# ultralytics/yolov5

Hardware: NVIDIA H100
Metric: images/sec @640 (forward + NMS) (higher is better)
Workload: dtype bf16

## Files before the change

### yolov5_b200/csrc/common.cuh

```cuda
#pragma once
#include <cuda.h>
#include <cuda_bf16.h>
#include <cuda_fp16.h>
#include <cuda_runtime.h>
#include <stdint.h>
#include <stdio.h>

namespace y5 {

__device__ __forceinline__ uint32_t smem_u32(const void* p) { return static_cast<uint32_t>(__cvta_generic_to_shared(p)); }

__device__ __forceinline__ bool elect_one() {
    uint32_t pred = 0;
    asm volatile(
        "{\n\t.reg .pred P;\n\t"
        "elect.sync _|P, 0xffffffff;\n\t"
        "selp.b32 %0, 1, 0, P;\n\t}"
        : "=r"(pred));
    return pred != 0;
}

__device__ __forceinline__ void mbar_init(uint64_t* bar, uint32_t count) {
    asm volatile("mbarrier.init.shared::cta.b64 [%0], %1;" ::"r"(smem_u32(bar)), "r"(count) : "memory");
}
__device__ __forceinline__ void fence_barrier_init() { asm volatile("fence.mbarrier_init.release.cluster;" ::: "memory"); }
__device__ __forceinline__ void fence_proxy_async_smem() { asm volatile("fence.proxy.async.shared::cta;" ::: "memory"); }

__device__ __forceinline__ void mbar_arrive(uint64_t* bar) {
    asm volatile("{\n\t.reg .b64 st;\n\tmbarrier.arrive.shared::cta.b64 st, [%0];\n\t}" ::"r"(smem_u32(bar)) : "memory");
}
__device__ __forceinline__ void mbar_arrive_expect_tx(uint64_t* bar, uint32_t bytes) {
    asm volatile("{\n\t.reg .b64 st;\n\tmbarrier.arrive.expect_tx.shared::cta.b64 st, [%0], %1;\n\t}" ::"r"(smem_u32(bar)),
                 "r"(bytes)
                 : "memory");
}
__device__ __forceinline__ bool mbar_try_wait(uint64_t* bar, uint32_t parity) {
    uint32_t ok;
    asm volatile(
        "{\n\t.reg .pred P;\n\t"
        "mbarrier.try_wait.parity.shared::cta.b64 P, [%1], %2;\n\t"
        "selp.b32 %0, 1, 0, P;\n\t}"
        : "=r"(ok)
        : "r"(smem_u32(bar)), "r"(parity)
        : "memory");
    return ok != 0;
}
__device__ __forceinline__ bool mbar_try_wait_hint(uint64_t* bar, uint32_t parity, uint32_t ns) {
    uint32_t ok;
    asm volatile(
        "{\n\t.reg .pred P;\n\t"
        "mbarrier.try_wait.parity.shared::cta.b64 P, [%1], %2, %3;\n\t"
        "selp.b32 %0, 1, 0, P;\n\t}"
        : "=r"(ok)
        : "r"(smem_u32(bar)), "r"(parity), "r"(ns)
        : "memory");
    return ok != 0;
}
__device__ __forceinline__ void mbar_wait(uint64_t* bar, uint32_t parity) {
    if (mbar_try_wait(bar, parity)) return;
    uint32_t spins = 0;
    while (!mbar_try_wait_hint(bar, parity, 20000u)) {
        if (++spins > 200000u) __trap();
    }
}

__device__ __forceinline__ void tma_prefetch_desc(const CUtensorMap* m) {
    asm volatile("prefetch.tensormap [%0];" ::"l"(reinterpret_cast<uint64_t>(m)) : "memory");
}
__device__ __forceinline__ void tma_load_2d(const CUtensorMap* m, uint64_t* bar, void* dst, int c0, int c1) {
    asm volatile(
        "cp.async.bulk.tensor.2d.shared::cluster.global.mbarrier::complete_tx::bytes [%0], [%1, {%3, %4}], [%2];" ::"r"(
            smem_u32(dst)),
        "l"(reinterpret_cast<uint64_t>(m)), "r"(smem_u32(bar)), "r"(c0), "r"(c1)
        : "memory");
}
__device__ __forceinline__ void tma_load_4d(const CUtensorMap* m, uint64_t* bar, void* dst, int c0, int c1, int c2, int c3) {
    asm volatile(
        "cp.async.bulk.tensor.4d.shared::cluster.global.mbarrier::complete_tx::bytes [%0], [%1, {%3, %4, %5, %6}], [%2];" ::"r"(
            smem_u32(dst)),
        "l"(reinterpret_cast<uint64_t>(m)), "r"(smem_u32(bar)), "r"(c0), "r"(c1), "r"(c2), "r"(c3)
        : "memory");
}
__device__ __forceinline__ void tma_load_2d_mcast(const CUtensorMap* m, uint64_t* bar, void* dst, int c0, int c1, uint16_t mask) {
    asm volatile(
        "cp.async.bulk.tensor.2d.shared::cluster.global.mbarrier::complete_tx::bytes.multicast::cluster"
        " [%0], [%1, {%3, %4}], [%2], %5;" ::"r"(smem_u32(dst)),
        "l"(reinterpret_cast<uint64_t>(m)), "r"(smem_u32(bar)), "r"(c0), "r"(c1), "h"(mask)
        : "memory");
}
__device__ __forceinline__ uint32_t mapa_u32(const void* p, uint32_t rank) {
    uint32_t r;
    asm volatile("mapa.shared::cluster.u32 %0, %1, %2;" : "=r"(r) : "r"(smem_u32(p)), "r"(rank));
    return r;
}
__device__ __forceinline__ void mbar_arrive_cluster(uint32_t bar_addr) {
    asm volatile("mbarrier.arrive.release.cluster.shared::cluster.b64 _, [%0];" ::"r"(bar_addr) : "memory");
}
__device__ __forceinline__ uint32_t cluster_ctarank() { uint32_t r; asm volatile("mov.u32 %0, %%cluster_ctarank;" : "=r"(r)); return r; }
__device__ __forceinline__ uint32_t cluster_nctarank() { uint32_t r; asm volatile("mov.u32 %0, %%cluster_nctarank;" : "=r"(r)); return r; }
__device__ __forceinline__ void cluster_sync_all() {
    asm volatile("barrier.cluster.arrive.release.aligned;" ::: "memory");
    asm volatile("barrier.cluster.wait.acquire.aligned;" ::: "memory");
}
__device__ __forceinline__ void tma_load_im2col_4d(const CUtensorMap* m, uint64_t* bar, void* dst, int c, int w, int h,
                                                   int n, uint16_t off_w, uint16_t off_h) {
    asm volatile(
        "cp.async.bulk.tensor.4d.shared::cluster.global.im2col.mbarrier::complete_tx::bytes"
        " [%0], [%1, {%3, %4, %5, %6}], [%2], {%7, %8};" ::"r"(smem_u32(dst)),
        "l"(reinterpret_cast<uint64_t>(m)), "r"(smem_u32(bar)), "r"(c), "r"(w), "r"(h), "r"(n), "h"(off_w), "h"(off_h)
        : "memory");
}
__device__ __forceinline__ void tma_store_2d(const CUtensorMap* m, const void* src, int c0, int c1) {
    asm volatile("cp.async.bulk.tensor.2d.global.shared::cta.bulk_group [%0, {%2, %3}], [%1];" ::"l"(
                     reinterpret_cast<uint64_t>(m)),
                 "r"(smem_u32(src)), "r"(c0), "r"(c1)
                 : "memory");
}
__device__ __forceinline__ void tma_store_4d(const CUtensorMap* m, const void* src, int c0, int c1, int c2, int c3) {
    asm volatile("cp.async.bulk.tensor.4d.global.shared::cta.bulk_group [%0, {%2, %3, %4, %5}], [%1];" ::"l"(
                     reinterpret_cast<uint64_t>(m)),
                 "r"(smem_u32(src)), "r"(c0), "r"(c1), "r"(c2), "r"(c3)
                 : "memory");
}
__device__ __forceinline__ void tma_store_commit() { asm volatile("cp.async.bulk.commit_group;" ::: "memory"); }
__device__ __forceinline__ void tma_store_wait_read0() { asm volatile("cp.async.bulk.wait_group.read 0;" ::: "memory"); }
__device__ __forceinline__ void tma_store_wait_all() { asm volatile("cp.async.bulk.wait_group 0;" ::: "memory"); }

__device__ __forceinline__ uint32_t gmma_desc_hi(uint32_t row_bytes) {
    const uint32_t layout = row_bytes == 128 ? 1u : (row_bytes == 64 ? 2u : 3u);
    return (((8u * row_bytes) >> 4) & 0x3FFFu) | (layout << 30);
}
__device__ __forceinline__ uint32_t gmma_desc_lo(uint32_t saddr) { return ((saddr >> 4) & 0x3FFFu) | (1u << 16); }
__device__ __forceinline__ uint64_t gmma_desc(uint32_t lo, uint32_t hi) { return (static_cast<uint64_t>(hi) << 32) | lo; }

__device__ __forceinline__ void wgmma_fence() { asm volatile("wgmma.fence.sync.aligned;" ::: "memory"); }
__device__ __forceinline__ void wgmma_commit() { asm volatile("wgmma.commit_group.sync.aligned;" ::: "memory"); }
template <int N>
__device__ __forceinline__ void wgmma_wait() { asm volatile("wgmma.wait_group.sync.aligned %0;" ::"n"(N) : "memory"); }
template <int N>
__device__ __forceinline__ void fence_regs(float (&d)[N]) {
#pragma unroll
    for (int i = 0; i < N; ++i) asm volatile("" : "+f"(d[i])::"memory");
}

template <uint32_t R>
__device__ __forceinline__ void setmaxnreg_dec() { asm volatile("setmaxnreg.dec.sync.aligned.u32 %0;" ::"n"(R)); }
template <uint32_t R>
__device__ __forceinline__ void setmaxnreg_inc() { asm volatile("setmaxnreg.inc.sync.aligned.u32 %0;" ::"n"(R)); }

__device__ __forceinline__ void griddep_wait() { asm volatile("griddepcontrol.wait;" ::: "memory"); }
__device__ __forceinline__ void griddep_launch_dependents() { asm volatile("griddepcontrol.launch_dependents;" ::: "memory"); }

__device__ __forceinline__ uint32_t ld_shared_u32(uint32_t addr) {
    uint32_t v;
    asm volatile("ld.shared.b32 %0, [%1];" : "=r"(v) : "r"(addr) : "memory");
    return v;
}
__device__ __forceinline__ void st_shared_u32(uint32_t addr, uint32_t v) {
    asm volatile("st.shared.b32 [%0], %1;" ::"r"(addr), "r"(v) : "memory");
}

__device__ __forceinline__ void named_bar_sync(uint32_t id, uint32_t nthreads) {
    asm volatile("bar.sync %0, %1;" ::"r"(id), "r"(nthreads) : "memory");
}

#ifndef Y5_SILU_EXACT
__device__ __forceinline__ float silu_f(float x) {
    const float h = 0.5f * x;
    float t;
    asm("tanh.approx.f32 %0, %1;" : "=f"(t) : "f"(h));
    return fmaf(h, t, h);
}
__device__ __forceinline__ float silu_from_half(float h) {
    float t;
    asm("tanh.approx.f32 %0, %1;" : "=f"(t) : "f"(h));
    return fmaf(h, t, h);
}
#else
__device__ __forceinline__ float silu_f(float x) { return __fdividef(x, 1.0f + __expf(-x)); }
// ... 36 lines not shown
```

### yolov5_b200/csrc/conv_gemm.cu

```cuda
#include <cmath>
#include <cstdio>
#include <cstdlib>
#include <cstring>
#include <mutex>
#include <type_traits>

#include "../../include/y5b200.h"
#include "common.cuh"
#include "host_util.h"
#include "wgmma.cuh"

namespace y5 {

constexpr int kBlockM = 128;
constexpr int kConsumers = 2;
constexpr int kConsumerThreads = 128 * kConsumers;
constexpr int kThreads = 128 + kConsumerThreads;
constexpr int kMaxStages = 8;
constexpr int kHeadN = 128;
constexpr int kHeadMaxNo = 8192;
constexpr int kHeadMaxNc = 4096;

__host__ __device__ inline int head_stage_cols(int no) { return no < kHeadN ? no : kHeadN; }

enum AMode { A_LINEAR = 0, A_IM2COL = 1, A_PATCH = 2 };

struct ConvParams {
    int M, N;
    int num_m_tiles;
    int num_m_super, num_n_tiles;
    int kh, kw, c_chunks;
    int block_k;
    int a_mode;
    int Ho, Wo, HoWo, stride, pad_h, pad_w;
    int tw, th, tiles_x, tiles_y;
    int b_grouped;
    int patch_pw;
    int cluster_n;
    uint32_t stg_bytes;
    int tma_epi;
    uint32_t b_sub_bytes;
    float rcp_per_img, rcp_tiles_x, rcp_HoWo, rcp_Wo;
    int a_stages, b_stages;
    uint32_t a_sub_bytes, a_stage_bytes, b_stage_bytes;
    int is_bf16, act;
    const float* bias;
    int bias_n;
    void* out;
    int out_pitch;
    const void* res;
    int res_pitch;
    void* raw;
    void* z;
    int na, no, nc, nx, z_rows, z_row0;
    float det_stride;
    float anchor_wh[8];
    float slope;
};

struct SmemLayout {
    uint32_t off_a, off_b, off_out, off_bias, off_bars, total;
};

__host__ __device__ inline SmemLayout smem_layout(int epi, int no, int bias_n, int a_stages, int b_stages, uint32_t a_bytes,
                                                   uint32_t b_bytes, uint32_t stg_bytes) {
    SmemLayout L;
    uint32_t o = 0;
    L.off_a = o;
    o += a_stages * a_bytes;
    L.off_b = o;
    o += b_stages * b_bytes;
    o = (o + 1023) & ~1023u;
    L.off_out = o;
    if (epi == 1) o += 4 * ((kBlockM * head_stage_cols(no) * 2 + 1023) & ~1023u);
    else o += stg_bytes;
    L.off_bias = o;
    o += ((bias_n + 3) & ~3) * 4;
    o = (o + 7) & ~7u;
    L.off_bars = o;
    o += (4 * kMaxStages + 2) * 8;
    L.total = o;
    return L;
}

__device__ __forceinline__ int fdiv(int n, int d, float rd) {
    if (n >= (1 << 23)) return n / d;
    int q = __float2int_rz(__int2float_rz(n) * rd);
    const int r = n - q * d;
    if (r >= d) ++q;
    else if (r < 0) --q;
    return q;
}

template <int BLOCK_N>
struct EpiBox {
    static constexpr int kRB = BLOCK_N * 2 < 128 ? BLOCK_N * 2 : 128;
    static constexpr int kCols = kRB / 2;
    static constexpr int kNB = BLOCK_N / kCols;
    static constexpr uint32_t kBytes = 64u * kRB;
};
struct EpiOrigin {
    int x, y, img;
};
__device__ __forceinline__ EpiOrigin epi_origin(const ConvParams& p, int mt, int wg) {
    if (p.a_mode != A_PATCH) return {0, mt * kBlockM + 64 * wg, 0};
    const int per_img = p.tiles_x * p.tiles_y;
    const int img = fdiv(mt, per_img, p.rcp_per_img);
    const int rem = mt - img * per_img;
    const int ty = fdiv(rem, p.tiles_x, p.rcp_tiles_x);
    const int x = (rem - ty * p.tiles_x) * p.tw, y = ty * p.th;
    return p.tw > 64 ? EpiOrigin{x + 64 * wg, y, img} : EpiOrigin{x, y + wg * (64 / p.tw), img};
}

template <int BLOCK_N, int MT, int KS, bool BF16>
__device__ __forceinline__ void mma_batch(float (&acc)[MT][BLOCK_N / 2], uint32_t a_lo, uint32_t a_sub16, uint32_t a_hi, uint32_t b_lo,
                                          uint32_t b_hi, uint32_t scale_first) {
    wgmma_fence();
#pragma unroll
    for (int k = 0; k < KS; ++k)
#pragma unroll
        for (int mi = 0; mi < MT; ++mi)
            Wgmma<BLOCK_N>::template run<BF16, 0, 0>(acc[mi], gmma_desc(a_lo + mi * a_sub16 + 2 * k, a_hi), gmma_desc(b_lo + 2 * k, b_hi),
                                                     k == 0 ? scale_first : 1u);
    wgmma_commit();
}

template <int BLOCK_N, int EPI, int MT, bool OPT, bool BF16>
__global__ void __launch_bounds__(kThreads, 1)
conv_gemm_kernel(const __grid_constant__ CUtensorMap tmA, const __grid_constant__ CUtensorMap tmB, const __grid_constant__ CUtensorMap tmO,
                 const __grid_constant__ CUtensorMap tmR, const ConvParams p) {
    static_assert(MT * BLOCK_N <= 256, "accumulators: at most 128 fp32 registers per consumer thread");
    constexpr bool kConv = EPI != 1;
    constexpr bool kLeaky = EPI == 2;
    constexpr int kAcc = BLOCK_N / 2;
    using Box = EpiBox<BLOCK_N>;
    const bool tma_epi = kConv && !OPT && p.tma_epi;

    extern __shared__ __align__(1024) uint8_t smem_raw[];
    uint8_t* smem = reinterpret_cast<uint8_t*>((reinterpret_cast<uintptr_t>(smem_raw) + 1023) & ~uintptr_t(1023));
    const SmemLayout L = smem_layout(EPI, p.no, p.bias_n, p.a_stages, p.b_stages, p.a_stage_bytes, p.b_stage_bytes, p.stg_bytes);
// ... 41 lines not shown
    griddep_launch_dependents();

    const int nn = p.num_n_tiles;
    const int num_tiles = ((p.num_m_super + csize - 1) / csize) * nn;
    const int tile0 = blockIdx.x / csize, tile_step = gridDim.x / csize;
    const uint32_t row_bytes = p.block_k * 2;
    const bool patch = p.a_mode == A_PATCH;
    const bool wide = OPT && p.patch_pw > 0;
    const int grp = wide ? p.kh * p.kw : (patch ? p.kh : 1);
    const int num_groups = wide ? p.c_chunks : (patch ? p.c_chunks * p.kw : p.kh * p.kw * p.c_chunks);

    if (warp < 4) {
        setmaxnreg_dec<56>();
    }
    if (warp == 0) {
        int as = 0, bs = 0;
        uint32_t aph = 0, bph = 0, sph = 0;
        for (int tile = tile0; tile < num_tiles; tile += tile_step) {
            const int ms = (tile / nn) * csize + static_cast<int>(crank);
            const int n0 = (tile - (tile / nn) * nn) * BLOCK_N;
            int img[MT], y0[MT], x0[MT];
#pragma unroll
            for (int mi = 0; mi < MT; ++mi) {
                const int mt = ms * MT + mi;
                img[mi] = y0[mi] = x0[mi] = 0;
                if (p.a_mode == A_IM2COL) {
                    const int m0 = mt * kBlockM;
                    img[mi] = fdiv(m0, p.HoWo, p.rcp_HoWo);
                    const int rem = m0 - img[mi] * p.HoWo;
                    const int oy = fdiv(rem, p.Wo, p.rcp_Wo);
                    y0[mi] = oy * p.stride - p.pad_h;
                    x0[mi] = (rem - oy * p.Wo) * p.stride - p.pad_w;
                } else if (patch) {
                    const int per_img = p.tiles_x * p.tiles_y;
                    img[mi] = fdiv(mt, per_img, p.rcp_per_img);
                    const int rem = mt - img[mi] * per_img;
                    const int ty = fdiv(rem, p.tiles_x, p.rcp_tiles_x);
                    y0[mi] = ty * p.th - p.pad_h;
                    x0[mi] = (rem - ty * p.tiles_x) * p.tw - p.pad_w;
                }
            }
            auto issue_group = [&](int cc, int s, int r0) {
                mbar_wait(&a_empty[as], aph ^ 1);
                if (elect_one()) {
                    mbar_arrive_expect_tx(&a_full[as], p.a_stage_bytes);
#pragma unroll
                    for (int mi = 0; mi < MT; ++mi) {
                        uint8_t* a_dst = sA + as * p.a_stage_bytes + mi * p.a_sub_bytes;
                        if (wide) {
                            if (mi == 0) tma_load_4d(&tmA, &a_full[as], a_dst, cc * p.block_k, x0[0], y0[0], img[0]);
                        } else if (p.a_mode == A_LINEAR) tma_load_2d(&tmA, &a_full[as], a_dst, cc * p.block_k, (ms * MT + mi) * kBlockM);
                        else if (p.a_mode == A_IM2COL)
                            tma_load_im2col_4d(&tmA, &a_full[as], a_dst, cc * p.block_k, x0[mi], y0[mi], img[mi], static_cast<uint16_t>(s),
                                               static_cast<uint16_t>(r0));
                        else tma_load_4d(&tmA, &a_full[as], a_dst, cc * p.block_k, x0[mi] + s, y0[mi], img[mi]);
                    }
                }
                __syncwarp();
                if (++as == p.a_stages) { as = 0; aph ^= 1; }
                for (int j = 0; j < grp; ++j) {
                    const int r = patch ? j : r0;
                    const int kb = wide ? j * p.c_chunks + cc : (r * p.kw + s) * p.c_chunks + cc;
                    const bool stage_first = !p.b_grouped || j == 0, stage_last = !p.b_grouped || j == grp - 1;
                    if (stage_first) mbar_wait(&b_empty[bs], bph ^ 1);
                    if (elect_one()) {
                        if (stage_first) mbar_arrive_expect_tx(&b_full[bs], p.b_stage_bytes);
                        uint8_t* b_dst = sB + bs * p.b_stage_bytes + (p.b_grouped ? j * p.b_sub_bytes : 0u);
                        if (csize == 1) tma_load_2d(&tmB, &b_full[bs], b_dst, kb * p.block_k, n0);
                        else {
                            const int slice_rows = BLOCK_N / csize;
                            tma_load_2d_mcast(&tmB, &b_full[bs], b_dst + crank * slice_rows * row_bytes, kb * p.block_k,
                                              n0 + static_cast<int>(crank) * slice_rows, static_cast<uint16_t>((1u << csize) - 1u));
                        }
                    }
                    __syncwarp();
                    if (stage_last && ++bs == p.b_stages) { bs = 0; bph ^= 1; }
                }
            };
            if (wide) {
                for (int cc = 0; cc < p.c_chunks; ++cc) issue_group(cc, 0, 0);
            } else if (patch) {
                for (int cc = 0; cc < p.c_chunks; ++cc)
                    for (int s = 0; s < p.kw; ++s) issue_group(cc, s, 0);
            } else {
                for (int r = 0; r < p.kh; ++r)
                    for (int s = 0; s < p.kw; ++s)
                        for (int cc = 0; cc < p.c_chunks; ++cc) issue_group(cc, s, r);
            }
            if (tma_epi) {
                mbar_wait(stg_free, sph ^ 1);
                if (elect_one()) {
                    if (p.res) {
                        mbar_arrive_expect_tx(res_full, p.stg_bytes);
#pragma unroll 1
                        for (int i = 0; i < kConsumers * MT; ++i) {
                            const EpiOrigin o = epi_origin(p, ms * MT + i % MT, i / MT);
#pragma unroll
                            for (int b = 0; b < Box::kNB; ++b) {
                                uint8_t* dst = stg + (i * Box::kNB + b) * Box::kBytes;
                                if (patch) tma_load_4d(&tmR, res_full, dst, n0 + b * Box::kCols, o.x, o.y, o.img);
                                else tma_load_2d(&tmR, res_full, dst, n0 + b * Box::kCols, o.y);
                            }
                        }
                    } else {
                        mbar_arrive(res_full);
                    }
                }
                __syncwarp();
                sph ^= 1;
            }
        }
    } else if (warp >= 4) {
    setmaxnreg_inc<224>();
    const int wg = (warp >> 2) - 1;
    const int ct = threadIdx.x - 128;
    const int wrow = wg * 64 + (warp & 3) * 16 + (lane >> 2);
    const int ccol = 2 * (lane & 3);
    const bool signal = (threadIdx.x & 127) == 0;
    constexpr bool bf16 = BF16;
    const uint32_t dhi = gmma_desc_hi(row_bytes);
    const uint32_t a_hi = wide ? (dhi & ~0x3FFFu) | (((static_cast<uint32_t>(p.patch_pw) * row_bytes) >> 4) & 0x3FFFu) : dhi;
    const uint32_t a_base = gmma_desc_lo(smem_u32(sA) + (wide ? wg * 8 * p.patch_pw : wg * 64) * row_bytes), b_base = gmma_desc_lo(smem_u32(sB));
    const uint32_t row16 = row_bytes >> 4;
    const uint32_t a_stage16 = p.a_stage_bytes >> 4, b_stage16 = p.b_stage_bytes >> 4, a_sub16 = p.a_sub_bytes >> 4;
    const uint32_t b_sub16 = p.b_sub_bytes >> 4;
    const uint32_t a_shift16 = patch ? (p.tw * row_bytes) >> 4 : 0;
    const int k_steps = p.block_k / 16;
    const int per_img = p.tiles_x * p.tiles_y;
    const int tw_shift = patch ? __ffs(p.tw) - 1 : 0;
    int as = 0, bs = 0, head_set = 0;
    uint32_t aph = 0, bph = 0, rph = 0;
    float acc[MT][kAcc];
#pragma unroll
    for (int mi = 0; mi < MT; ++mi)
#pragma unroll
        for (int i = 0; i < kAcc; ++i) acc[mi][i] = 0.0f;

    int pend_as = 0, pend_bs = 0;
    bool pend_a_last = false, pend_b_last = false;
    auto release_pending = [&]() {
        if (!signal) return;
        if (pend_b_last) {
            if (csize == 1) mbar_arrive(&b_empty[pend_bs]);
            else
                for (int r = 0; r < csize; ++r) mbar_arrive_cluster(mapa_u32(&b_empty[pend_bs], static_cast<uint32_t>(r)));
        }
        if (pend_a_last) mbar_arrive(&a_empty[pend_as]);
    };

    for (int tile = tile0; tile < num_tiles; tile += tile_step) {
        const int ms = (tile / nn) * csize + static_cast<int>(crank);
        const int nt = tile - (tile / nn) * nn;
        const int n0 = nt * BLOCK_N;
        for (int g = 0; g < num_groups; ++g) {
            mbar_wait(&a_full[as], aph);
            const uint32_t a_stage_lo = a_base + as * a_stage16;
            uint32_t a_lo = a_stage_lo;
            for (int j = 0; j < grp; ++j) {
                if (wide) {
                    const int tr = j / p.kw, ts = j - tr * p.kw;
                    a_lo = a_stage_lo + (tr * p.patch_pw + ts) * row16;
                }
                const bool stage_first = !p.b_grouped || j == 0, stage_last = !p.b_grouped || j == grp - 1;
                if (stage_first) mbar_wait(&b_full[bs], bph);
                const uint32_t b_lo = b_base + bs * b_stage16 + (p.b_grouped ? j * b_sub16 : 0u);
                const uint32_t scale_first = (g | j) != 0 ? 1u : 0u;
// ... 458 lines not shown
    g.pad_w = d->kw ? d->pad_w : d->pad;
    g.xs = d->in_x_stride ? d->in_x_stride : d->in_pitch;
    g.ys = d->in_y_stride ? d->in_y_stride : static_cast<long long>(d->in_w) * g.xs;
    g.ns = d->in_n_stride ? d->in_n_stride : static_cast<long long>(d->in_h) * g.ys;
    g.Ho = (d->in_h + 2 * g.pad_h - g.kh) / d->stride + 1;
    g.Wo = (d->in_w + 2 * g.pad_w - g.kw) / d->stride + 1;
    return g;
}

int encode_epi_map(CUtensorMap* map, int dtype, const void* base, int pitch, const ConvParams& p, int batch, int bn, const char* what) {
    const int rb = bn * 2 < 128 ? bn * 2 : 128;
    const cuuint64_t px = static_cast<cuuint64_t>(pitch) * 2;
    if (p.a_mode == A_PATCH) {
        cuuint64_t dims[4] = {(cuuint64_t)p.N, (cuuint64_t)p.Wo, (cuuint64_t)p.Ho, (cuuint64_t)batch};
        cuuint64_t str[3] = {px, px * p.Wo, px * p.HoWo};
        cuuint32_t box[4] = {(cuuint32_t)(rb / 2), (cuuint32_t)(p.tw < 64 ? p.tw : 64), (cuuint32_t)(p.tw < 64 ? 64 / p.tw : 1), 1};
        return encode_tiled(map, dtype, base, 4, dims, str, box, swizzle_for_row_bytes(rb), what);
    }
    cuuint64_t dims[2] = {(cuuint64_t)p.N, (cuuint64_t)p.M};
    cuuint64_t str[1] = {px};
    cuuint32_t box[2] = {(cuuint32_t)(rb / 2), 64};
    return encode_tiled(map, dtype, base, 2, dims, str, box, swizzle_for_row_bytes(rb), what);
}

}

struct y5_conv_plan {
    PlanCommon pc;
};
struct y5_detect_plan {
    PlanCommon pc;
};

extern "C" Y5_API int y5_conv_pick(int32_t in_c, int32_t out_c, int64_t m_rows, int32_t* block_k, int32_t* block_n) {
    if (in_c <= 0 || out_c <= 0) return set_error(Y5_E_INVALID, "y5_conv_pick: non-positive channel count");
    if (block_k) *block_k = pick_block_k(in_c);
    if (block_n) *block_n = pick_block_n(out_c, m_rows);
    return 0;
}

static int validate_conv(const y5_conv_desc* d) {
    if (!d || !d->in || !d->weight || !d->bias || !d->out) return set_error(Y5_E_INVALID, "conv: null pointer");
    if (d->dtype != Y5_F16 && d->dtype != Y5_BF16) return set_error(Y5_E_UNSUPPORTED, "conv: dtype must be fp16/bf16");
    if (d->batch <= 0 || d->in_h <= 0 || d->in_w <= 0 || d->in_c <= 0 || d->out_c <= 0)
        return set_error(Y5_E_INVALID, "conv: non-positive dimension");
    const long long xs = d->in_x_stride ? d->in_x_stride : d->in_pitch;
    if (xs <= 0 || xs % 8 || (d->in_y_stride % 8) || (d->in_n_stride % 8) || d->out_pitch < d->out_c || d->out_pitch % 8 || d->out_c % 8)
        return set_error(Y5_E_INVALID, "conv: strides/pitches/out_c must be multiples of 8 elements and cover the view");
    if (!d->in_x_stride && d->in_pitch < d->in_c) return set_error(Y5_E_INVALID, "conv: in_pitch smaller than in_c");
    if (!aligned16(d->in) || !aligned16(d->out) || !aligned16(d->weight) || (d->residual && !aligned16(d->residual)))
        return set_error(Y5_E_INVALID, "conv: pointers must be 16-byte aligned");
    if (d->residual && (d->res_pitch < d->out_c || d->res_pitch % 8)) return set_error(Y5_E_INVALID, "conv: bad residual pitch");
    if (d->act != Y5_ACT_NONE && d->act != Y5_ACT_SILU && d->act != Y5_ACT_LEAKY)
        return set_error(Y5_E_UNSUPPORTED, "conv: activation code %d unsupported", d->act);
    if (d->act == Y5_ACT_LEAKY && !std::isfinite(d->act_slope)) return set_error(Y5_E_INVALID, "conv: LeakyReLU slope must be finite");
    const int kw = d->kw ? d->kw : d->ksize, pw = d->kw ? d->pad_w : d->pad;
    if (d->ksize < 1 || d->ksize > 7 || kw < 1 || kw > 7 || d->stride < 1 || d->stride > 8 || d->pad < 0 || d->pad > d->ksize || pw < 0 ||
        pw > kw)
        return set_error(Y5_E_UNSUPPORTED, "conv: kernel %dx%d stride %d pad %d,%d unsupported", d->ksize, kw, d->stride, d->pad, pw);
    return 0;
}

extern "C" Y5_API int y5_conv_plan_create(const y5_conv_desc* d, y5_conv_plan** out) {
    if (!out) return set_error(Y5_E_INVALID, "conv: null plan out");
    *out = nullptr;
    if (int e = validate_conv(d)) return e;
    const Geo g = geometry(d);
    if (g.Ho <= 0 || g.Wo <= 0) return set_error(Y5_E_INVALID, "conv: empty output");
    const int64_t M64 = static_cast<int64_t>(d->batch) * g.Ho * g.Wo;
    if (M64 > 0x7fffffff - 256) return set_error(Y5_E_UNSUPPORTED, "conv: more than 2^31 output pixels");
    const int bk = d->block_k ? d->block_k : pick_block_k(d->in_c);
    if (bk != 16 && bk != 32 && bk != 64) return set_error(Y5_E_INVALID, "conv: block_k must be 16/32/64");
    const bool plain = g.kh == 1 && g.kw == 1 && d->stride == 1 && g.pad_h == 0 && g.pad_w == 0 && !d->in_x_stride && !d->in_y_stride &&
                       !d->in_n_stride;
    int best_tw = 0;
    double best_eff = 0.0;
    if (d->stride == 1 && !plain) {
        for (int tw = 8; tw <= 128; tw <<= 1) {
            const int th = 128 / tw;
            const double eff = (double)g.Wo * g.Ho / ((double)((g.Wo + tw - 1) / tw * tw) * ((g.Ho + th - 1) / th * th));
            if (eff > best_eff + 1e-9) { best_eff = eff; best_tw = tw; }
        }
    }
    int a_mode_sel;
    if (plain) a_mode_sel = A_LINEAR;
    else if (d->a_mode == 2 && d->stride != 1) return set_error(Y5_E_INVALID, "conv: patch mode needs stride 1");
    else if (d->a_mode == 2 || (d->a_mode == 0 && d->stride == 1 && best_eff >= 0.75)) a_mode_sel = A_PATCH;
    else a_mode_sel = A_IM2COL;

    int bn = d->block_n, mt_sel = 0, cl_sel = 1;
    {
        int bn_auto = 0;
        pick_tile(d->out_c, (M64 + kBlockM - 1) / kBlockM, &bn_auto, &mt_sel);
        if (!bn) bn = bn_auto;
        else {
            mt_sel = bn < 128 ? 128 / bn : ((d->reserved & 2) && bn == 128 ? 2 : 1);
            cl_sel = (d->reserved >> 8) > 1 ? (d->reserved >> 8) : 1;
            if (d->reserved & 4) cl_sel = 2;
            if (cl_sel != 1 && cl_sel != 2 && cl_sel != 4) return set_error(Y5_E_INVALID, "conv: cluster size must be 1, 2 or 4");
        }
    }
    if (bn != 32 && bn != 64 && bn != 128 && bn != 256) return set_error(Y5_E_INVALID, "conv: block_n must be 32/64/128/256");
    auto* plan = new y5_conv_plan();
    PlanCommon& pc = plan->pc;
    std::memset(&pc.p, 0, sizeof(pc.p));
    ConvParams& p = pc.p;
    p.M = static_cast<int>(M64);
    p.N = d->out_c;
    p.kh = g.kh; p.kw = g.kw;
    p.Ho = g.Ho; p.Wo = g.Wo; p.HoWo = g.Ho * g.Wo;
    p.rcp_HoWo = 1.0f / static_cast<float>(p.HoWo);
    p.rcp_Wo = 1.0f / static_cast<float>(p.Wo);
    p.stride = d->stride;
    p.pad_h = g.pad_h; p.pad_w = g.pad_w;
    p.is_bf16 = d->dtype == Y5_BF16;
    p.act = d->act == Y5_ACT_SILU;
    p.slope = d->act_slope;
    p.bias = d->bias;
    p.out = d->out;
    p.out_pitch = d->out_pitch;
    p.res = d->residual;
    p.res_pitch = d->res_pitch;
    p.block_k = bk;
    p.c_chunks = (d->in_c + bk - 1) / bk;
    const int row_bytes = bk * 2;
    p.b_sub_bytes = bn * row_bytes;
    p.b_stage_bytes = p.b_sub_bytes;
    p.a_mode = a_mode_sel;

    const CUtensorMapSwizzle sw = swizzle_for_row_bytes(row_bytes);
    int e = 0;
    if (p.a_mode == A_LINEAR) {
        p.num_m_tiles = (p.M + kBlockM - 1) / kBlockM;
        p.a_sub_bytes = kBlockM * row_bytes;
        cuuint64_t dims[2] = {(cuuint64_t)d->in_c, (cuuint64_t)p.M};
        cuuint64_t str[1] = {(cuuint64_t)d->in_pitch * 2};
        cuuint32_t box[2] = {(cuuint32_t)bk, kBlockM};
        e = encode_tiled(&pc.tmA, d->dtype, d->in, 2, dims, str, box, sw, "A linear");
    } else if (p.a_mode == A_IM2COL) {
        p.num_m_tiles = (p.M + kBlockM - 1) / kBlockM;
        p.a_sub_bytes = kBlockM * row_bytes;
        e = encode_im2col(&pc.tmA, d->dtype, d->in, d->in_c, d->in_w, d->in_h, d->batch, g.xs, g.ys, g.ns, g.kh, g.kw, d->stride, g.pad_h,
                          g.pad_w, bk, kBlockM, sw);
    } else {
        p.tw = best_tw;
        p.th = 128 / best_tw;
        {
            const int tx8 = (g.Wo + 7) / 8, ty16 = (g.Ho + 15) / 16;
            const double eff8 = (double)g.Wo * g.Ho / ((double)tx8 * 8 * ty16 * 16);
            if ((d->reserved & 128) && !(d->reserved & 32) && row_bytes == 128 && g.kw > 1 && (mt_sel == 1 || (mt_sel == 2 && tx8 % 2 == 0)) &&
                eff8 >= best_eff - 1e-9) {
                p.tw = 8;
                p.th = 16;
                p.patch_pw = 8 * mt_sel + 8;
            }
        }
        if (!p.patch_pw && g.kh > 1 && bn <= 128) {
            p.b_grouped = 1;
            p.b_stage_bytes = g.kh * p.b_sub_bytes;
        }
        p.tiles_x = (g.Wo + p.tw - 1) / p.tw;
        p.tiles_y = (g.Ho + p.th - 1) / p.th;
        p.rcp_tiles_x = 1.0f / static_cast<float>(p.tiles_x);
        p.rcp_per_img = 1.0f / static_cast<float>(p.tiles_x * p.tiles_y);
        p.num_m_tiles = d->batch * p.tiles_x * p.tiles_y;
        p.a_sub_bytes = p.patch_pw ? 8 * row_bytes : (p.th + g.kh - 1) * p.tw * row_bytes;
        cuuint64_t dims[4] = {(cuuint64_t)d->in_c, (cuuint64_t)d->in_w, (cuuint64_t)d->in_h, (cuuint64_t)d->batch};
        cuuint64_t str[3] = {(cuuint64_t)g.xs * 2, (cuuint64_t)g.ys * 2, (cuuint64_t)g.ns * 2};
        cuuint32_t box[4] = {(cuuint32_t)bk, (cuuint32_t)(p.patch_pw ? p.patch_pw : p.tw), (cuuint32_t)(p.th + g.kh - 1), 1};
        e = encode_tiled(&pc.tmA, d->dtype, d->in, 4, dims, str, box, sw, "A patch");
    }
    if (e) { delete plan; return e; }
    const uint64_t ktot = static_cast<uint64_t>(p.kh) * p.kw * p.c_chunks * bk;
    {
        cuuint64_t dims[2] = {ktot, (cuuint64_t)d->out_c};
        cuuint64_t str[1] = {ktot * 2};
        cuuint32_t box[2] = {(cuuint32_t)bk, (cuuint32_t)(bn / cl_sel)};
        e = encode_tiled(&pc.tmB, d->dtype, d->weight, 2, dims, str, box, sw, "B");
    }
    if (e) { delete plan; return e; }
    const bool opt_modes = cl_sel > 1 || p.patch_pw > 0 || (d->reserved & 8);
    const bool stages_first = p.a_mode == A_IM2COL && bn == 256;
    if (!(d->reserved & 16) && !opt_modes && !stages_first) {
        p.tma_epi = 1;
        p.stg_bytes = static_cast<uint32_t>(mt_sel * bn * 256);
        e = encode_epi_map(&pc.tmO, d->dtype, d->out, d->out_pitch, p, d->batch, bn, "output");
        if (!e && d->residual) e = encode_epi_map(&pc.tmR, d->dtype, d->residual, d->res_pitch, p, d->batch, bn, "residual");
        if (e) { delete plan; return e; }
    } else if ((d->reserved & 8) && !(d->reserved & 16)) {
        p.stg_bytes = static_cast<uint32_t>(kConsumers * 64 * (bn * 2 + 16));
    }
    const int epi = d->act == Y5_ACT_LEAKY ? 2 : 0;
    int e2 = finish_plan(pc, bn, epi, mt_sel, cl_sel);
    if (e2 && p.stg_bytes) {
        p.stg_bytes = 0;
        p.tma_epi = 0;
        e2 = finish_plan(pc, bn, epi, mt_sel, cl_sel);
    }
    if (e2) { delete plan; return e2; }
    *out = plan;
    return 0;
}

extern "C" Y5_API int y5_conv_plan_run(const y5_conv_plan* plan, void* stream) {
    if (!plan) return set_error(Y5_E_INVALID, "conv: null plan");
    return run_plan(plan->pc, static_cast<cudaStream_t>(stream));
}
extern "C" Y5_API void y5_conv_plan_destroy(y5_conv_plan* plan) { delete plan; }

extern "C" Y5_API int y5_conv_plan_info(const y5_conv_plan* plan, struct y5_conv_plan_info* out) {
    if (!plan || !out) return set_error(Y5_E_INVALID, "conv: null plan/info");
// ... 115 lines not shown
```

### yolov5_b200/engine.py

```python
from __future__ import annotations

import ctypes as C
import math
import os
from collections import namedtuple

import torch

from . import _lib
from ._lib import ConvDesc, DetectDesc, WgradDesc
from .models.common import (C3Ghost, TransformerBlock, check_grouped_convs, ghost_bottleneck_convs, ghost_dw_channels, pool_modes, spp_kernel,
                            transformer_spec)

BN_EPS_DEFAULT = 1e-3
HEAD_N = 128
HEAD_MAX_NO = 8192
HEAD_MAX_NC = 4096


class View:

    __slots__ = ("buf", "coff", "c", "h", "w")

    def __init__(self, buf: torch.Tensor, coff: int, c: int):
        self.buf, self.coff, self.c = buf, coff, c
        self.h, self.w = buf.shape[1], buf.shape[2]

    @property
    def pitch(self) -> int:
        return self.buf.shape[3]

    @property
    def ptr(self) -> int:
        return self.buf.data_ptr() + self.coff * self.buf.element_size()

    def slice(self, coff: int, c: int) -> "View":
        assert 0 <= coff and coff + c <= self.c
        return View(self.buf, self.coff + coff, c)

    def dense_nhwc(self) -> torch.Tensor:
        return self.buf[..., self.coff : self.coff + self.c]


def _pad8(c: int) -> int:
    return (c + 7) // 8 * 8


def fold_conv_bn(conv: torch.nn.Conv2d, bn) -> tuple[torch.Tensor, torch.Tensor]:
    w = conv.weight.detach().float()
    if bn is None:
        b = conv.bias.detach().float() if conv.bias is not None else torch.zeros(w.shape[0], device=w.device)
        return w, b
    scale = bn.weight.detach().float() / torch.sqrt(bn.running_var.detach().float() + bn.eps)
    w2 = w * scale.view(-1, 1, 1, 1)
    b0 = conv.bias.detach().float() if conv.bias is not None else torch.zeros_like(scale)
    b2 = bn.bias.detach().float() + (b0 - bn.running_mean.detach().float()) * scale
    return w2, b2


def pack_weight(w: torch.Tensor, block_k: int, dtype: torch.dtype) -> torch.Tensor:
    o, i, kh, kw = w.shape
    cin_pad = (i + block_k - 1) // block_k * block_k
    out = torch.zeros(o, kh, kw, cin_pad, dtype=dtype, device=w.device)
    out[..., :i] = w.permute(0, 2, 3, 1).to(dtype)
    return out.contiguous()


def stem_weight_s2d(w: torch.Tensor) -> torch.Tensor:
    o = w.shape[0]
    out = torch.zeros(o, 16, 3, 3, dtype=w.dtype, device=w.device)
    for dy in range(2):
        for dx in range(2):
            for c in range(3):
                out[:, (dy * 2 + dx) * 3 + c] = w[:, c, dy::2, dx::2]
    return out


def stem_weight_wide(w3: torch.Tensor) -> torch.Tensor:
    return w3.permute(0, 3, 1, 2).reshape(w3.shape[0], 48, 3, 1)


def stem_weight_narrow(wv: torch.Tensor) -> torch.Tensor:
    return wv.view(wv.shape[0], 3, 16, 3).permute(0, 2, 3, 1)


def stem_buffer(b: int, h: int, w: int, dtype: torch.dtype, device) -> torch.Tensor:
    return torch.zeros(b, h // 2, w // 2 + 2, 16, dtype=dtype, device=device)


def stem_s2d(img: torch.Tensor, out: torch.Tensor) -> None:
    b, _, h, w = img.shape
    row = out.shape[2]
    img = img.contiguous()
    _lib.check(_lib.lib().y5_stem_s2d(img.data_ptr(), _lib.dtype_code(img.dtype), out.data_ptr(), _lib.dtype_code(out.dtype), b, h, w, row,
                                      (row - w // 2) // 2, C.c_void_p(_lib.stream_ptr(out.device))), "stem_s2d")


IMAGE_C = 16


def image_nhwc(img: torch.Tensor, out: torch.Tensor) -> None:
    b, _, h, w = img.shape
    img = img.contiguous()
    _lib.check(_lib.lib().y5_image_nhwc(img.data_ptr(), _lib.dtype_code(img.dtype), out.data_ptr(), _lib.dtype_code(out.dtype), b, h, w,
                                        out.shape[3], C.c_void_p(_lib.stream_ptr(out.device))), "image_nhwc")


def pad_image_weight(w: torch.Tensor) -> torch.Tensor:
    return torch.nn.functional.pad(w, (0, 0, 0, 0, 0, IMAGE_C - w.shape[1]))


_block_k_cache: dict = {}


def block_k(cin: int, cout: int, m_rows: int) -> int:
    key = (cin, cout, m_rows)
    v = _block_k_cache.get(key)
    if v is None:
        bk = C.c_int32()
        _lib.check(_lib.lib().y5_conv_pick(cin, cout, m_rows, C.byref(bk), None), "conv_pick")
        v = _block_k_cache[key] = bk.value
    return v


def is_v6_stem(m) -> bool:
    c = m.conv
    return c.kernel_size[0] == 6 and c.stride[0] == 2 and c.padding[0] == 2 and c.in_channels == 3


def act_spec(act: torch.nn.Module) -> tuple[int, float]:
    if isinstance(act, torch.nn.SiLU):
        return _lib.ACT_SILU, 0.0
    if isinstance(act, torch.nn.Identity):
        return _lib.ACT_NONE, 0.0
    if isinstance(act, torch.nn.ReLU):
        return _lib.ACT_LEAKY, 0.0
    if isinstance(act, torch.nn.LeakyReLU) and math.isfinite(act.negative_slope):
        return _lib.ACT_LEAKY, float(act.negative_slope)
    raise NotImplementedError(f"y5b200: activation {act!r} (SiLU, ReLU, LeakyReLU and Identity are built)")


ConvInput = namedtuple("ConvInput", "inp in_pitch batch in_h in_w in_c kw pad_w in_x_stride in_y_stride in_n_stride", defaults=(0,) * 5)


def stem_geom(buf: torch.Tensor, wide: bool) -> ConvInput:
    b, h2, row, _ = buf.shape
    geom = dict(in_pitch=16, batch=b, in_h=h2, in_w=row - 2, in_x_stride=16, in_y_stride=row * 16, in_n_stride=h2 * row * 16)
    if wide:
        return ConvInput(inp=buf.data_ptr(), in_c=48, kw=1, pad_w=0, **geom)
    return ConvInput(inp=buf.data_ptr() + 16 * buf.element_size(), in_c=16, kw=3, pad_w=1, **geom)


def conv_desc(x: ConvInput, wp: torch.Tensor, bias: torch.Tensor, bk: int, out: int, out_pitch: int, k: int, s: int, p: int,
              act: bool | tuple[int, float], dtype: torch.dtype, residual: int | None = None, res_pitch: int = 0) -> ConvDesc:
    d = ConvDesc()
    d.inp, d.in_pitch, d.batch, d.in_h, d.in_w, d.in_c, d.kw, d.pad_w, d.in_x_stride, d.in_y_stride, d.in_n_stride = x
    d.weight, d.bias = wp.data_ptr(), bias.data_ptr()
    d.out, d.out_pitch, d.out_c = out, out_pitch, wp.shape[0]
    d.residual, d.res_pitch = residual, res_pitch
    d.ksize, d.stride, d.pad = k, s, p
    d.act, d.act_slope = act if isinstance(act, tuple) else (_lib.ACT_SILU if act else _lib.ACT_NONE, 0.0)
    d.dtype, d.block_k = _lib.dtype_code(dtype), bk
    return d


def wgrad_desc(x: ConvInput, dy: int, dy_pitch: int, dw: torch.Tensor, k: int, s: int, p: int, dtype: torch.dtype) -> WgradDesc:
    d = WgradDesc()
    d.inp, d.in_pitch, d.batch, d.in_h, d.in_w, d.in_c, d.kw, d.pad_w, d.in_x_stride, d.in_y_stride, d.in_n_stride = x
    d.dout, d.dout_pitch, d.out_c = dy, dy_pitch, dw.shape[0]
    d.dweight = dw.data_ptr()
    d.ksize, d.stride, d.pad = k, s, p
    d.dtype = _lib.dtype_code(dtype)
    return d


class _Op:

    __slots__ = ("fn", "args", "name", "keep")

    def __init__(self, name, fn, args, keep=()):
        self.name, self.fn, self.args, self.keep = name, fn, args, keep

    def run(self, stream: int):
        _lib.check(self.fn(*self.args, C.c_void_p(stream)), self.name)


class Program:

    def __init__(self, module, batch: int, height: int, width: int, dtype: torch.dtype, device, in_channels=None):
        if dtype not in (torch.float16, torch.bfloat16):
            raise TypeError(f"y5b200 engine computes in fp16 or bf16, got {dtype} (call model.half() / .bfloat16())")
        self.lib = _lib.lib()
        self.module = module
        self.B, self.H, self.W = batch, height, width
        self.dtype, self.device = dtype, torch.device(device)
        self.dt_code = _lib.dtype_code(dtype)
        self.ops: list[_Op] = []
        self.head_ops: list = []
        self._plans: list = []
        self._keep: list = []
        self.graph = None
        self.flops = 0
        self.act_bytes = 0
        self.weight_bytes = 0
        self.in_channels = in_channels
        self._build()

    def new_buf(self, h: int, w: int, c: int) -> torch.Tensor:
        t = torch.zeros(self.B, h, w, _pad8(c), dtype=self.dtype, device=self.device)
        self._keep.append(t)
        return t

    def new_view(self, h: int, w: int, c: int) -> View:
        return View(self.new_buf(h, w, c), 0, c)

    def fold_pack(self, parts, m_rows: int):
        cin, kh, kw = parts[0][0].shape[1:]
        cout = sum(w.shape[0] for w, _, _ in parts)
        bk = block_k(cin, cout, m_rows)
        ipad = (cin + bk - 1) // bk * bk
        wp = torch.empty(cout, kh, kw, ipad, dtype=self.dtype, device=self.device)
        bias = torch.empty(cout, dtype=torch.float32, device=self.device)
        self.fold_pack_into(parts, wp, bias, 0, ipad)
        return wp, bias, bk

    def fold_pack_into(self, parts, wp, bias, row0: int, ipad: int, pad_rows_to: int | None = None):
        st = C.c_void_p(_lib.stream_ptr(self.device))
        es = wp.element_size()
        for w, cb, bn in parts:
            w = w.detach()
            if not w.is_contiguous():
                w = w.contiguous()
            if w.device != self.device:
# ... 383 lines not shown
        outs: list = [None] * n
        x = None
        for i, m in enumerate(layers):
            f = m.f
            name = f"model.{i}"
            if isinstance(m, (my.Detect,)):
                xs = [outs[j] for j in f]
                if isinstance(m, my.Segment):
                    self.proto_view = self.lower_proto(m.proto, xs[0], f"{name}.proto")
                self.lower_detect(m, xs, name)
                continue
            if isinstance(m, mc.Classify):
                self.lower_classify(m, outs[i - 1] if f == -1 else (outs[f] if isinstance(f, int) else [outs[j] for j in f]), name)
                continue
            if isinstance(m, mc.Concat):
                cat = concat_buf[i]
                off = 0
                for j in f:
                    src = i - 1 if j == -1 else j
                    v = outs[src]
                    want = cat.slice(off, v.c)
                    if not (v.buf is cat.buf and v.coff == want.coff):
                        self.copy_into(v, want, f"{name}.copy{src}")
                    off += v.c
                outs[i] = cat
                continue
            xin = (torch.empty(0) if i == 0 else outs[i - 1]) if f == -1 else outs[f % i]
            if isinstance(m, torch.nn.ZeroPad2d):
                outs[i] = xin
            elif isinstance(m, torch.nn.MaxPool2d):
                outs[i] = self.lower_pool(xin, assigned.get(i), pools[i], name)
            else:
                outs[i] = self._lower(m, xin, assigned.get(i), name)
        self.outs = outs

    def _shape_of(self, m, src):
        from .models import common as mc
        from .models import yolo as my

        if isinstance(m, mc.Conv):
            c, h, w = src
            k, s, p = m.conv.kernel_size[0], m.conv.stride[0], m.conv.padding[0]
            return (m.conv.out_channels, (h + 2 * p - k) // s + 1, (w + 2 * p - k) // s + 1)
        if isinstance(m, mc.C3):
            return (m.cv3.conv.out_channels, src[1], src[2])
        if isinstance(m, (mc.SPPF, mc.SPP, mc.Bottleneck)):
            return (m.cv2.conv.out_channels, src[1], src[2])
        if isinstance(m, mc.GhostConv):
            c, h, w = src
            k, s, p = m.cv1.conv.kernel_size[0], m.cv1.conv.stride[0], m.cv1.conv.padding[0]
            return (2 * m.cv1.conv.out_channels, (h + 2 * p - k) // s + 1, (w + 2 * p - k) // s + 1)
        if isinstance(m, mc.GhostBottleneck):
            return (2 * m.conv[2].cv1.conv.out_channels, src[1], src[2])
        if isinstance(m, torch.nn.Sequential):
            for sub in m:
                src = self._shape_of(sub, src)
            return src
        if isinstance(m, torch.nn.ZeroPad2d):
            left, right, top, bottom = m.padding
            return (src[0], src[1] + top + bottom, src[2] + left + right)
        if isinstance(m, torch.nn.MaxPool2d):
            s = m.stride if isinstance(m.stride, int) else m.stride[0]
            return (src[0], (src[1] - 2) // s + 1, (src[2] - 2) // s + 1)
        if isinstance(m, torch.nn.Upsample):
            return (src[0], src[1] * 2, src[2] * 2)
        if isinstance(m, mc.Concat):
            return (sum(s[0] for s in src), src[0][1], src[0][2])
        if isinstance(m, (my.Detect, mc.Classify)):
            return None
        raise NotImplementedError(f"y5b200: module {type(m).__name__} is outside the engine's hot path")

    def _run_fixed(self, stream: int):
        for op in self.ops:
            op.run(stream)

    def capture(self):
        s = torch.cuda.Stream(device=self.device)
        s.wait_stream(torch.cuda.current_stream(self.device))
        with torch.cuda.stream(s):
            self._run_fixed(s.cuda_stream)
        torch.cuda.current_stream(self.device).wait_stream(s)
        torch.cuda.synchronize(self.device)
        g = torch.cuda.CUDAGraph()
        with torch.cuda.graph(g, stream=s):
            self._run_fixed(torch.cuda.current_stream(self.device).cuda_stream)
        self.graph = g

    def _run_body(self, img: torch.Tensor, use_graph: bool) -> int:
        assert img.is_cuda and img.shape == (self.B, 3, self.H, self.W), (img.shape, (self.B, 3, self.H, self.W))
        if self.image_in is not None:
            image_nhwc(img, self.image_in)
        else:
            stem_s2d(img, self.stem_in)
        st = _lib.stream_ptr(self.device)
        if use_graph and os.environ.get("Y5_NO_GRAPH") != "1":
            if self.graph is None:
                self.capture()
            self.graph.replay()
        else:
            self._run_fixed(st)
        return st

    def run_classify(self, img: torch.Tensor, use_graph: bool = True) -> torch.Tensor:
        st = self._run_body(img, use_graph)
        v = self.cls_view
        y = torch.empty(self.B, v.c, dtype=self.dtype, device=self.device)
        _lib.check(self.lib.y5_nhwc_to_nchw(v.ptr, v.pitch, y.data_ptr(), self.B, 1, 1, v.c, self.dt_code, C.c_void_p(st)), "nhwc_to_nchw")
        return y

    def run_model(self, img: torch.Tensor, use_graph: bool = True):
        st = self._run_body(img, use_graph)
        no = self.det_shapes[0][-1]
        z = torch.empty(self.B, self.z_rows, no, dtype=self.dtype, device=self.device)
        raws = [torch.empty(s, dtype=self.dtype, device=self.device) for s in self.det_shapes]
        for plan, raw in zip(self.head_ops, raws):
            _lib.check(self.lib.y5_detect_plan_run_to(plan, raw.data_ptr(), z.data_ptr(), C.c_void_p(st)), "detect")
        proto = None
        if self.proto_view is not None:
            pv = self.proto_view
            proto = torch.empty(self.B, pv.c, pv.h, pv.w, dtype=self.dtype, device=self.device)
            _lib.check(self.lib.y5_nhwc_to_nchw(pv.ptr, pv.pitch, proto.data_ptr(), self.B, pv.h, pv.w, pv.c, self.dt_code,
                                                C.c_void_p(st)), "nhwc_to_nchw")
        return z, raws, proto

    def run_layer(self, x: torch.Tensor) -> torch.Tensor:
        v = self.layer_in
        v.buf[..., : v.c].copy_(x.permute(0, 2, 3, 1))
        st = _lib.stream_ptr(self.device)
        self._run_fixed(st)
        o = self.single_out
        y = torch.empty(self.B, o.c, o.h, o.w, dtype=self.dtype, device=self.device)
        _lib.check(self.lib.y5_nhwc_to_nchw(o.ptr, o.pitch, y.data_ptr(), self.B, o.h, o.w, o.c, self.dt_code, C.c_void_p(st)),
                   "nhwc_to_nchw")
        return y

    def launches_per_forward(self) -> int:
        n = len(self.ops) + len(self.head_ops) + (1 if self.stem_in is not None or self.image_in is not None else 0)
        n += 1 if self.proto_view is not None else 0
        return n + (1 if self.cls_view is not None else 0)

    def __del__(self):
        try:
            for fn, h in self._plans:
                fn(h)
        except Exception:
            pass
```

### yolov5_b200/utils/torch_utils.py

```python
from __future__ import annotations

import ctypes as C
import math
import os
from copy import deepcopy

import torch
from torch import nn

from .. import _lib


def fuse_conv_and_bn(conv: nn.Conv2d, bn: nn.BatchNorm2d) -> nn.Conv2d:
    fused = nn.Conv2d(conv.in_channels, conv.out_channels, conv.kernel_size, conv.stride, conv.padding, conv.dilation,
                      conv.groups, bias=True).requires_grad_(False).to(conv.weight.device, conv.weight.dtype)
    scale = bn.weight / torch.sqrt(bn.running_var + bn.eps)
    fused.weight.copy_(conv.weight * scale.view(-1, 1, 1, 1))
    b0 = conv.bias if conv.bias is not None else torch.zeros_like(scale)
    fused.bias.copy_(bn.bias + (b0 - bn.running_mean) * scale)
    return fused


def smartCrossEntropyLoss(label_smoothing=0.0):
    from .loss import CrossEntropyLoss
# ... 405 lines not shown
        raise NotImplementedError(f"y5b200: optimizer {name} is outside the hot path (train.py offers SGD, Adam and AdamW)")
    g = [], [], []
    bn = tuple(v for k, v in nn.__dict__.items() if "Norm" in k)
    for v in model.modules():
        for p_name, p in v.named_parameters(recurse=False):
            if p_name == "bias":
                g[2].append(p)
            elif p_name == "weight" and isinstance(v, bn):
                g[1].append(p)
            else:
                g[0].append(p)
    if name == "Adam":
        opt = FusedAdam(g[2], lr=lr, betas=(momentum, 0.999))
    elif name == "AdamW":
        opt = FusedAdamW(g[2], lr=lr, betas=(momentum, 0.999), weight_decay=0.0)
    else:
        opt = FusedSGD(g[2], lr=lr, momentum=momentum, nesterov=True)
    opt.add_param_group({"params": g[0], "weight_decay": decay})
    opt.add_param_group({"params": g[1], "weight_decay": 0.0})
    return opt


class GraphedTrainStep:

    def __init__(self, model, compute_loss, optimizer, batch: int, size, max_targets: int | None = None, amp_dtype=torch.float16,
                 max_norm: float | None = 10.0, warmup_steps: int = 3, ema=None, init_scale: float = 65536.0):
        if not isinstance(optimizer, _FusedOptimizer):
            raise TypeError("GraphedTrainStep needs a fused optimizer (yolov5_b200.utils.torch_utils.smart_optimizer / FusedSGD / FusedAdam): its "
                            "overflow-skipping step is what makes the loss-scaled update capturable")
        dev = next(model.parameters()).device
        h, w = (size, size) if isinstance(size, int) else size
        self.max_targets = max_targets or 64 * batch
        self.img = torch.zeros(batch, 3, h, w, dtype=torch.uint8, device=dev)
        self.tgt = torch.zeros(self.max_targets, 6, dtype=torch.float32, device=dev)
        self.items = torch.zeros(3, dtype=torch.float32, device=dev)
        self.optimizer, self.max_norm = optimizer, max_norm
        self.scaler = torch.amp.GradScaler("cuda", init_scale=init_scale, enabled=amp_dtype == torch.float16)
        scaler = self.scaler
        if isinstance(model, (nn.parallel.DataParallel, nn.parallel.DistributedDataParallel)):
            raise TypeError("GraphedTrainStep: pass the plain module; for data parallel use FusedSGD.data_parallel(model), whose single "
                            "all-reduce is capturable")
        world = optimizer._dp[1] if optimizer._dp is not None else 1

        from .. import train_ops

        syncing = [n for n, m in model.named_modules() if train_ops.bn_process_group(m) is not None]
        if syncing:
            raise NotImplementedError(f"GraphedTrainStep: {len(syncing)} SyncBatchNorm layers (first: {syncing[0]}) all-reduce their batch "
                                      "statistics inside the forward and backward, which this step does not capture; train such a model "
                                      "with the eager step, or convert it back to BatchNorm2d")

        def step():
            with torch.autocast("cuda", dtype=amp_dtype):
                pred = model(self.img)
            loss, items = compute_loss(pred, self.tgt)
            if world > 1:
                loss = loss * world
            prev = train_ops.set_async_wgrad(os.environ.get("Y5_ASYNC_WGRAD", "1") != "0")
            try:
                scaler.scale(loss).backward()
            finally:
                train_ops.set_async_wgrad(prev)
                train_ops.finish_async(dev)
            optimizer.fused_step(scaler=scaler, max_norm=max_norm, ema=ema, model=model)
            optimizer.zero_grad(set_to_none=True)
            self.items.copy_(items)

        lrs = [g["lr"] for g in optimizer.param_groups]
        state = {k: v.clone() for k, v in model.state_dict().items()}
        ema_state = {k: v.clone() for k, v in ema.ema.state_dict().items()} if ema is not None else None
        ema_updates = ema.updates if ema is not None else 0
        side = torch.cuda.Stream(dev)
        side.wait_stream(torch.cuda.current_stream(dev))
        with torch.cuda.stream(side):
            for g in optimizer.param_groups:
                g["lr"] = 0.0
            for _ in range(warmup_steps):
                step()
        torch.cuda.current_stream(dev).wait_stream(side)
        torch.cuda.synchronize(dev)
        for g, lr in zip(optimizer.param_groups, lrs):
            g["lr"] = lr
        self.graph = torch.cuda.CUDAGraph()
        with torch.cuda.graph(self.graph, capture_error_mode="thread_local" if world > 1 else "global"):
            step()
        self._arena_buf = train_ops._arena.buf
        self._pack_plans = list(model.__dict__.get("_y5_pack_plans", {}).values())
        model.load_state_dict(state)
        optimizer.zero_state()
        if ema is not None:
            ema.ema.load_state_dict(ema_state)
            ema.updates = ema_updates
            ema.hyper_init(optimizer._hyper)
        if self.scaler.is_enabled():
            self.scaler._scale.fill_(init_scale)
            self.scaler._growth_tracker.zero_()
        self.ema = ema

    def __call__(self, imgs_u8: torch.Tensor, targets: torch.Tensor) -> torch.Tensor:
        nt = targets.shape[0]
        if nt > self.max_targets:
            raise ValueError(f"GraphedTrainStep: {nt} label rows > max_targets {self.max_targets}")
        self.img.copy_(imgs_u8, non_blocking=True)
        self.tgt.zero_()
        if nt:
            self.tgt[:nt].copy_(targets, non_blocking=True)
        self.optimizer.fill_hyper_host(self.max_norm)
        self.graph.replay()
        if self.ema is not None:
            self.ema.updates += 1
        return self.items
```

Before: 3181.

## Gate patch mode on A-heavy tiles, add patch K-order for im2col, relax cluster arrive

Patch A-mode is now used only when the M tile extent is at least the N tile, which should favour B-heavy layers with plain im2col. Those fallback im2col convs get a new K iteration order (channel chunk, then kw, then kh) meant to improve locality of the A loads. The cluster mbarrier arrive drops its explicit release.cluster qualifier to make it cheaper, which risks memory-ordering bugs if the default semantics are weaker. Garbage collection is also disabled during CUDA graph capture, which affects capture only and not steady-state replay.

```diff
diff --git a/yolov5_b200/csrc/common.cuh b/yolov5_b200/csrc/common.cuh
--- a/yolov5_b200/csrc/common.cuh
+++ b/yolov5_b200/csrc/common.cuh
@@ -94,7 +94,7 @@
     return r;
 }
 __device__ __forceinline__ void mbar_arrive_cluster(uint32_t bar_addr) {
-    asm volatile("mbarrier.arrive.release.cluster.shared::cluster.b64 _, [%0];" ::"r"(bar_addr) : "memory");
+    asm volatile("mbarrier.arrive.shared::cluster.b64 _, [%0];" ::"r"(bar_addr) : "memory");
 }
 __device__ __forceinline__ uint32_t cluster_ctarank() { uint32_t r; asm volatile("mov.u32 %0, %%cluster_ctarank;" : "=r"(r)); return r; }
 __device__ __forceinline__ uint32_t cluster_nctarank() { uint32_t r; asm volatile("mov.u32 %0, %%cluster_nctarank;" : "=r"(r)); return r; }
diff --git a/yolov5_b200/csrc/conv_gemm.cu b/yolov5_b200/csrc/conv_gemm.cu
--- a/yolov5_b200/csrc/conv_gemm.cu
+++ b/yolov5_b200/csrc/conv_gemm.cu
@@ -56,6 +56,7 @@
     float det_stride;
     float anchor_wh[8];
     float slope;
+    int k_patch_order;
 };
 
 struct SmemLayout {
@@ -263,6 +264,10 @@
             } else if (patch) {
                 for (int cc = 0; cc < p.c_chunks; ++cc)
                     for (int s = 0; s < p.kw; ++s) issue_group(cc, s, 0);
+            } else if (p.k_patch_order) {
+                for (int cc = 0; cc < p.c_chunks; ++cc)
+                    for (int s = 0; s < p.kw; ++s)
+                        for (int r = 0; r < p.kh; ++r) issue_group(cc, s, r);
             } else {
                 for (int r = 0; r < p.kh; ++r)
                     for (int s = 0; s < p.kw; ++s)
@@ -887,11 +892,18 @@
             if (eff > best_eff + 1e-9) { best_eff = eff; best_tw = tw; }
         }
     }
+    bool a_heavy = true;
+    if (!d->block_n) {
+        int bn_t = 0, mt_t = 0;
+        pick_tile(d->out_c, (M64 + kBlockM - 1) / kBlockM, &bn_t, &mt_t);
+        a_heavy = mt_t * kBlockM >= bn_t;
+    }
     int a_mode_sel;
     if (plain) a_mode_sel = A_LINEAR;
     else if (d->a_mode == 2 && d->stride != 1) return set_error(Y5_E_INVALID, "conv: patch mode needs stride 1");
-    else if (d->a_mode == 2 || (d->a_mode == 0 && d->stride == 1 && best_eff >= 0.75)) a_mode_sel = A_PATCH;
+    else if (d->a_mode == 2 || (d->a_mode == 0 && d->stride == 1 && best_eff >= 0.75 && a_heavy)) a_mode_sel = A_PATCH;
     else a_mode_sel = A_IM2COL;
+    const bool k_patch_order = a_mode_sel == A_IM2COL && d->a_mode == 0 && d->stride == 1 && best_eff >= 0.75;
 
     int bn = d->block_n, mt_sel = 0, cl_sel = 1;
     {
@@ -932,6 +944,7 @@
     p.b_sub_bytes = bn * row_bytes;
     p.b_stage_bytes = p.b_sub_bytes;
     p.a_mode = a_mode_sel;
+    p.k_patch_order = k_patch_order;
 
     const CUtensorMapSwizzle sw = swizzle_for_row_bytes(row_bytes);
     int e = 0;
diff --git a/yolov5_b200/engine.py b/yolov5_b200/engine.py
--- a/yolov5_b200/engine.py
+++ b/yolov5_b200/engine.py
@@ -1,6 +1,8 @@
 from __future__ import annotations
 
+import contextlib
 import ctypes as C
+import gc
 import math
 import os
 from collections import namedtuple
@@ -149,6 +151,18 @@
     if wide:
         return ConvInput(inp=buf.data_ptr(), in_c=48, kw=1, pad_w=0, **geom)
     return ConvInput(inp=buf.data_ptr() + 16 * buf.element_size(), in_c=16, kw=3, pad_w=1, **geom)
+
+
+@contextlib.contextmanager
+def no_collection_during_capture():
+    gc.collect()
+    was_enabled = gc.isenabled()
+    gc.disable()
+    try:
+        yield
+    finally:
+        if was_enabled:
+            gc.enable()
 
 
 def conv_desc(x: ConvInput, wp: torch.Tensor, bias: torch.Tensor, bk: int, out: int, out_pitch: int, k: int, s: int, p: int,
@@ -698,7 +712,7 @@
         torch.cuda.current_stream(self.device).wait_stream(s)
         torch.cuda.synchronize(self.device)
         g = torch.cuda.CUDAGraph()
-        with torch.cuda.graph(g, stream=s):
+        with no_collection_during_capture(), torch.cuda.graph(g, stream=s):
             self._run_fixed(torch.cuda.current_stream(self.device).cuda_stream)
         self.graph = g
 
diff --git a/yolov5_b200/utils/torch_utils.py b/yolov5_b200/utils/torch_utils.py
--- a/yolov5_b200/utils/torch_utils.py
+++ b/yolov5_b200/utils/torch_utils.py
@@ -511,7 +511,9 @@
         for g, lr in zip(optimizer.param_groups, lrs):
             g["lr"] = lr
         self.graph = torch.cuda.CUDAGraph()
-        with torch.cuda.graph(self.graph, capture_error_mode="thread_local" if world > 1 else "global"):
+        from ..engine import no_collection_during_capture
+
+        with no_collection_during_capture(), torch.cuda.graph(self.graph, capture_error_mode="thread_local" if world > 1 else "global"):
             step()
         self._arena_buf = train_ops._arena.buf
         self._pack_plans = list(model.__dict__.get("_y5_pack_plans", {}).values())
```

New measurement: 3200, median of 6. Within noise of the previous version (+0.6%).
